# maxilevi/vits.cpp

Hardware: AMD Instinct MI355X
Metric: audio samples/sec end-to-end (ids -> fp32 PCM in HBM), vits-english architecture, batch=64 x 128 ids (higher is better)
Workload: dtype f32; 1 GPU; c3 b64x128 ref-mode f32 predicted-dur | vits-english = MMS-TTS arch, synthetic weights; batch_per_gpu=64, ids_per_utterance=128, parallelism=utterance-sharded x1

## Files before the change

### vits.cpp_amd/csrc/conv_mfma.hip

```cpp
#include <hip/hip_runtime.h>
#include <type_traits>

#include <algorithm>
#include <atomic>
#include <cmath>
#include <cstdint>
#include <cstdlib>
#include <cstring>

#include "kernels.h"

#ifndef VITS_CONV_PART
#define VITS_CONV_PART 0
#endif

namespace vits {

typedef float floatx16 __attribute__((ext_vector_type(16)));

constexpr int CK = 32;

struct ConvParams {
    const float* x;
    int64_t x_bs;
// ... 973 lines not shown
    const int t = t0 + col;
    if (EPI == EPI_STD) {
        float* yb = p.y + (int64_t)b * p.y_bs;
        float* y2b = p.y2 ? p.y2 + (int64_t)b * p.y_bs : nullptr;
        const float* rb = p.res ? p.res + (int64_t)b * p.r_bs : nullptr;
        const float* ab = p.acc ? p.acc + (int64_t)b * p.a_bs : nullptr;
#pragma unroll
        for (int r = 0; r < 4; ++r) {
            const int co = mtile * 32 + 16 * half + 4 * jg + r;
            if (co >= p.cout || t >= ncols) continue;
            float v = acc[r] + ep_bias[r];
            if (p.post_act == 1) v = v > 0.f ? v : 0.f;
            if (rb) v = ep_res[r] + v;
            if (ab) {
                v = ep_acc[r] + v;
                v = p.scale_div ? v / p.scale : v * p.scale;
            }
            if (p.post_act == 2) v = fmaxf(v, v * p.post_slope);
            yb[(int64_t)co * p.y_cs + t] = v;
            if (y2b) y2b[(int64_t)co * p.y_cs + t] = fmaxf(v, v * p.post_slope);
        }
    } else {
        float* ex = xs + (wm >> 1) * 256;
        __syncthreads();
        if (wm & 1) {
#pragma unroll
            for (int r = 0; r < 4; ++r) ex[r * 64 + lane] = acc[r];
        }
        __syncthreads();
        if (wm & 1) return;
        float* yb = p.y + (int64_t)b * p.y_bs;
        const int halfc = p.cout / 2;
#pragma unroll
        for (int r = 0; r < 4; ++r) {
            const int ch = (int)blockIdx.y * 32 + 16 * half + 4 * jg + r;
            if (ch >= halfc || t >= ncols) continue;
            yb[(int64_t)ch * p.y_cs + t] = wavenet_gate(acc[r] + ep_bias[r], ex[r * 64 + lane] + ep_b1[r]);
        }
    }
}

static int lat16_pitch(int span) { return span <= 4 ? 24 : span <= 20 ? 40 : span <= 52 ? 72 : 0; }
static hipError_t launch_lat16(const PackedConv& w, const ConvParams& p0, int ncols_max, int batch, hipStream_t s) {
    ConvParams p = p0;
    const int span = (w.kt - 1) * p.dil;
    const int pitch = lat16_pitch(span);
    if (!pitch || !w.wp_l16) return hipErrorInvalidValue;
    p.l16_fill4 = (reinterpret_cast<uintptr_t>(p.x) & 15) == 0 && (p.x_cs & 3) == 0 && (p.x_bs & 3) == 0;
    p.xw = pitch;
    p.kt_rt = w.kt;
    p.wl16 = w.wp_l16;
    size_t lds = ((size_t)w.nchunks + 1) * CK * pitch * sizeof(float);
    if (p.ln_gamma) lds += ((size_t)2 * 16 * 32 + 2 * (size_t)w.cin) * sizeof(float);
    dim3 grid((ncols_max + 15) / 16, (w.mtiles_used + 1) / 2, batch);
#define VITS_L16(E, PP)                                                                                                                          \
    do {                                                                                                                                         \
        static BigLdsOnce big;                                                                                                                   \
        if (lds > 64 * 1024 && big.needed()) {                                                                                                   \
            if (hipError_t e = hipFuncSetAttribute(reinterpret_cast<const void*>(&conv_lat16_kernel<E, PP>), hipFuncAttributeMaxDynamicSharedMemorySize, 160 * 1024)) \
                return e;                                                                                                                        \
            big.done();                                                                                                                          \
        }                                                                                                                                        \
        VITS_KLAUNCH((conv_lat16_kernel<E, PP>), grid, dim3(256), lds, s, p);                                                                    \
    } while (0)
    if (w.epi == EPI_GATE) {
        if (pitch != 24) return hipErrorInvalidValue;
        VITS_L16(EPI_GATE, 24);
    } else if (pitch == 24) {
        VITS_L16(EPI_STD, 24);
    } else if (pitch == 40) {
        VITS_L16(EPI_STD, 40);
    } else {
        VITS_L16(EPI_STD, 72);
    }
#undef VITS_L16
    return hipGetLastError();
}
#endif

struct ConvGroupParams {
    ConvParams m[3];
    int zend[3];
};
template <int DIL>
__global__ __launch_bounds__(320) VITS_WAVES_ATTR void conv_group_kernel(const ConvGroupParams g) {
    extern __shared__ __attribute__((aligned(16))) float xs_dyn[];
    const int z = blockIdx.z;
    if (z < g.zend[0]) conv_mfma_body<11, DIL, true, 2, 2, 2, 2, EPI_STD>(g.m[0], xs_dyn, blockIdx.x, blockIdx.y, z);
    else if (z < g.zend[1]) conv_mfma_body<7, DIL, true, 2, 2, 2, 2, EPI_STD>(g.m[1], xs_dyn, blockIdx.x, blockIdx.y, z - g.zend[0]);
    else conv_mfma_body<3, DIL, true, 2, 2, 2, 2, EPI_STD>(g.m[2], xs_dyn, blockIdx.x, blockIdx.y, z - g.zend[1]);
}

hipError_t make_conv_params(const PackedConv& w, const ConvCall& c, int tile, ConvParams& p);
struct TileShape {
    int wm, wn, mr, nr;
};
static TileShape tile_shape(int tile) {
    switch (tile) {
        case TILE_128x128: return {2, 2, 2, 2};
        case TILE_64x256: return {1, 4, 2, 2};
        case TILE_32x256: return {1, 4, 1, 2};
        case TILE_64x64: return {1, 4, 2, 1};
        case TILE_LAT16:
        case TILE_NARROW: return {4, 1, 1, 1};
        default: return {1, 4, 1, 1};
    }
}

#if VITS_CONV_PART == 0
int choose_conv_tile(int rows, int epi, int t_hint) {
    const int narrow = kernel_knobs().narrow_tiles;
    const bool small_t = t_hint <= 128 || (narrow && rows <= narrow);
    if (epi == EPI_GATE) return small_t ? TILE_64x64 : TILE_64x256;
    const int t128 = kernel_knobs().tile128;
    if (rows % 128 == 0 && t128) return TILE_128x128;
    if (rows % 64 == 0) return small_t ? TILE_64x64 : TILE_64x256;
    return small_t ? TILE_32x64 : TILE_32x256;
}

std::vector<float> pack_conv_weights(const float* w, int cout, int cin, int k, int epi, int ct_stride, int* rows_out, int* mtiles_used_out,
                                     int* mtiles_out, int* nchunks_out) {
    const int bm_tiles = 4;
    const int half = cout / 2;
    int rows, kt;
    if (epi == EPI_CONVT) {
        rows = cout * ct_stride;
        kt = k / ct_stride;
    } else {
        rows = cout;
        kt = k;
    }
    int mtiles = (rows + 31) / 32;
    if (epi == EPI_GATE) mtiles = 2 * ((half + 31) / 32);
    *mtiles_used_out = mtiles;
    mtiles = (mtiles + bm_tiles - 1) / bm_tiles * bm_tiles;
    const int nchunks = (cin + CK - 1) / CK;
    std::vector<float> out((size_t)mtiles * nchunks * kt * (CK / 2) * 64, 0.f);
    for (int mt = 0; mt < mtiles; ++mt)
        for (int c = 0; c < nchunks; ++c)
            for (int j = 0; j < kt; ++j)
                for (int pr = 0; pr < CK / 2; ++pr)
                    for (int l = 0; l < 64; ++l) {
                        const int ci = c * CK + 2 * pr + (l >> 5);
                        const int r = l & 31;
                        float v = 0.f;
                        if (ci < cin) {
                            if (epi == EPI_STD) {
                                const int co = mt * 32 + r;
                                if (co < cout) v = w[((size_t)co * cin + ci) * k + j];
                            } else if (epi == EPI_GATE) {
                                const int ch = (mt / 2) * 32 + r;
                                const int co = (mt & 1) ? half + ch : ch;
                                if (ch < half) v = w[((size_t)co * cin + ci) * k + j];
                            } else {
                                const int rho = mt * 32 + r;
                                const int co = rho / ct_stride, ph = rho % ct_stride;
                                if (co < cout) v = w[((size_t)ci * cout + co) * k + ph + ct_stride * j];
                            }
                        }
                        const size_t idx = (((((size_t)mt * nchunks + c) * kt + j) * (CK / 8) + pr / 4) * 64 + l) * 4 + (pr & 3);
                        out[idx] = v;
                    }
    *rows_out = rows;
    *mtiles_out = mtiles;
    *nchunks_out = nchunks;
    return out;
}

bool conv_lat16_candidate(int epi, int kt, int cin) {
    return (epi == EPI_STD || (epi == EPI_GATE && kt == 5)) && (int64_t)kt * cin >= 64;
}

std::vector<float> repack_conv_weights_l16(const std::vector<float>& packed, int mtiles, int nchunks, int kt) {
    std::vector<float> out(packed.size() + 32 * 256, 0.f);
    const size_t G = (size_t)nchunks * kt;
    for (int mt = 0; mt < mtiles; ++mt)
        for (int half = 0; half < 2; ++half)
            for (size_t g = 0; g < G; ++g)
                for (int hq = 0; hq < 2; ++hq)
                    for (int l = 0; l < 64; ++l)
                        for (int sc = 0; sc < 4; ++sc) {
                            const int ci = 16 * hq + 4 * sc + (l >> 4);
                            const int pr = ci >> 1, par = ci & 1;
                            const size_t src = (((((size_t)mt * G + g) * (CK / 8)) + pr / 4) * 64 + (16 * half + (l & 15) + 32 * par)) * 4 + (pr & 3);
                            const size_t dst = (((((size_t)mt * 2 + half) * (2 * G)) + 2 * g + hq) * 64 + l) * 4 + sc;
                            out[dst] = packed[src];
                        }
    return out;
}

#endif

template <int KT, int DIL, bool DB, int EPI>
static hipError_t launch_tile(const PackedConv& w, int tile, const ConvParams& p, int ncols_max, int batch, hipStream_t s) {
    const TileShape ts = tile_shape(tile);
    const int bn = ts.wn * ts.nr * 32;
    const int bm_tiles = ts.wm * ts.mr;
    dim3 grid((ncols_max + bn - 1) / bn, (w.mtiles_used + bm_tiles - 1) / bm_tiles, batch);
    const size_t lds = DB ? (size_t)p.nbuf * CK * ((p.xw + 3 + VITS_XWP_GRAN - 1) / VITS_XWP_GRAN * VITS_XWP_GRAN) * sizeof(float) : (size_t)CK * p.xw * sizeof(float);
#define VITS_LAUNCH(WM, WN, MR, NR)                                                                                                   \
    do {                                                                                                                              \
        static BigLdsOnce big_lds_set;          \
        if (lds > 64 * 1024 && big_lds_set.needed()) {                                                                                        \
            hipError_t ea = hipFuncSetAttribute(reinterpret_cast<const void*>(&conv_mfma_kernel<KT, DIL, DB, WM, WN, MR, NR, EPI>),       \
                                                hipFuncAttributeMaxDynamicSharedMemorySize, 160 * 1024);                             \
            if (ea != hipSuccess) return ea;                                                                                          \
            big_lds_set.done();                                                                                                 \
        }                                                                                                                             \
        VITS_KLAUNCH((conv_mfma_kernel<KT, DIL, DB, WM, WN, MR, NR, EPI>), grid, dim3(DB ? 320 : 256), lds, s, p);                             \
    } while (0)
    switch (tile) {
        case TILE_128x128:
            if (EPI == EPI_GATE) return hipErrorInvalidValue;
            VITS_LAUNCH(2, 2, 2, 2);
            break;
        case TILE_64x256: VITS_LAUNCH(1, 4, 2, 2); break;
        case TILE_64x64: VITS_LAUNCH(1, 4, 2, 1); break;
        case TILE_32x256:
            if (EPI == EPI_GATE) return hipErrorInvalidValue;
            VITS_LAUNCH(1, 4, 1, 2);
            break;
        case TILE_NARROW:
            if constexpr (DB && DIL == 1 && ((EPI == EPI_STD && KT <= 3) || (EPI == EPI_GATE && KT == 5))) {
                VITS_LAUNCH(4, 1, 1, 1);
                break;
            } else {
                return hipErrorInvalidValue;
            }
        default:
            if (EPI == EPI_GATE) return hipErrorInvalidValue;
            VITS_LAUNCH(1, 4, 1, 1);
            break;
    }
#undef VITS_LAUNCH
    return hipGetLastError();
}

#define VITS_GO(K, D, E)                                                                     \
    do {                                                                                     \
        if ((D) != 0 && db) return launch_tile<K, D, (D) != 0, E>(w, tile, p, ncols_max, batch, s); \
        return launch_tile<K, D, false, E>(w, tile, p, ncols_max, batch, s);                 \
    } while (0)
#define VITS_LAUNCHER(K) hipError_t launch_conv_k##K(const PackedConv& w, int tile, const ConvParams& p, int ncols_max, int batch, hipStream_t s, bool db)
VITS_LAUNCHER(3);
VITS_LAUNCHER(7);
VITS_LAUNCHER(11);
#if VITS_CONV_PART == 1
VITS_LAUNCHER(3) {
    if (p.dil == 1) VITS_GO(3, 1, EPI_STD);
    if (p.dil == 3) VITS_GO(3, 3, EPI_STD);
    if (p.dil == 5) VITS_GO(3, 5, EPI_STD);
    VITS_GO(3, 0, EPI_STD);
}
#endif
#if VITS_CONV_PART == 2
VITS_LAUNCHER(7) {
    if (p.dil == 1) VITS_GO(7, 1, EPI_STD);
    if (p.dil == 3) VITS_GO(7, 3, EPI_STD);
    if (p.dil == 5) VITS_GO(7, 5, EPI_STD);
    VITS_GO(7, 0, EPI_STD);
}
#endif
#if VITS_CONV_PART == 3
VITS_LAUNCHER(11) {
    if (p.dil == 1) VITS_GO(11, 1, EPI_STD);
    if (p.dil == 3) VITS_GO(11, 3, EPI_STD);
    if (p.dil == 5) VITS_GO(11, 5, EPI_STD);
    VITS_GO(11, 0, EPI_STD);
}
#endif

#if VITS_CONV_PART == 4
bool conv_group_supported(const PackedConv& w, int dil) {
    return w.epi == EPI_STD && (w.kt == 11 || w.kt == 7 || w.kt == 3) && (dil == 1 || dil == 3 || dil == 5) && w.rows % 128 == 0 && w.cin % CK == 0;
}
hipError_t launch_conv_group(const PackedConv* const* w, const ConvCall* c, int n, hipStream_t s) {
    if (n < 1 || n > 3) return hipErrorInvalidValue;
    ConvGroupParams g;
    std::memset(&g, 0, sizeof(g));
    const int slot_kt[3] = {11, 7, 3};
    int have[3] = {-1, -1, -1};
    for (int i = 0; i < n; ++i) {
        if (!conv_group_supported(*w[i], c[i].dil) || c[i].dil != c[0].dil || c[i].batch != c[0].batch || w[i]->rows != w[0]->rows || c[i].tile >= 0) return hipErrorInvalidValue;
        const int slot = w[i]->kt == 11 ? 0 : w[i]->kt == 7 ? 1 : 2;
        if (have[slot] >= 0) return hipErrorInvalidValue;
        have[slot] = i;
    }
    int z = 0, ncols_max = 0;
    size_t lds = 0;
    for (int slot = 0; slot < 3; ++slot) {
        if (have[slot] >= 0) {
            const int i = have[slot];
            if (hipError_t e = make_conv_params(*w[i], c[i], TILE_128x128, g.m[slot])) return e;
            if (g.m[slot].oneshot) return hipErrorInvalidValue;
            if (g.m[slot].bias_rows) return hipErrorInvalidValue;
            g.m[slot].nbuf = 2;
            z += c[i].batch;
            ncols_max = std::max(ncols_max, c[i].t_out);
            const int xwp = (g.m[slot].xw + 3 + VITS_XWP_GRAN - 1) / VITS_XWP_GRAN * VITS_XWP_GRAN;
            lds = std::max(lds, (size_t)2 * CK * xwp * sizeof(float));
        }
        g.zend[slot] = z;
        (void)slot_kt;
    }
    dim3 grid((ncols_max + 127) / 128, w[0]->mtiles_used / 4, z);
#define VITS_GROUP_LAUNCH(D)                                                                                                              \
    do {                                                                                                                                  \
        static BigLdsOnce big_lds_set;                                                                                      \
        if (lds > 64 * 1024 && big_lds_set.needed()) {                                                            \
            hipError_t ea = hipFuncSetAttribute(reinterpret_cast<const void*>(&conv_group_kernel<D>), hipFuncAttributeMaxDynamicSharedMemorySize, 160 * 1024); \
            if (ea != hipSuccess) return ea;                                                                                              \
            big_lds_set.done();                                                                           \
        }                                                                                                                                 \
        VITS_KLAUNCH((conv_group_kernel<D>), grid, dim3(320), lds, s, g);                                                           \
    } while (0)
    if (c[0].dil == 1) VITS_GROUP_LAUNCH(1);
    else if (c[0].dil == 3) VITS_GROUP_LAUNCH(3);
    else VITS_GROUP_LAUNCH(5);
#undef VITS_GROUP_LAUNCH
    return hipGetLastError();
}
#endif

#if VITS_CONV_PART == 0
int resolve_conv_tile(const PackedConv& w, const ConvCall& c) {
    const int ncols_max = w.epi == EPI_CONVT ? c.t_in + 1 : c.t_out;
    int tile = c.tile >= 0 ? c.tile : choose_conv_tile(w.rows, w.epi, ncols_max);
    if (c.tile < 0 && w.epi == EPI_GATE) {
        const TileShape t2 = tile_shape(tile);
        const int64_t nb = (ncols_max + t2.wn * t2.nr * 32 - 1) / (t2.wn * t2.nr * 32);
        if (nb * ((w.mtiles_used + 1) / 2) * c.batch < 512) tile = TILE_64x64;
    }
    if (c.tile < 0 && w.epi != EPI_GATE) {
        auto blocks = [&](int tl) {
            const TileShape t2 = tile_shape(tl);
            const int64_t nb = (ncols_max + t2.wn * t2.nr * 32 - 1) / (t2.wn * t2.nr * 32);
            const int64_t mb = (w.mtiles_used + t2.wm * t2.mr - 1) / (t2.wm * t2.mr);
            return nb * mb * c.batch;
        };
        const int64_t min_blocks_env = kernel_knobs().min_blocks;
        const int64_t min_blocks = min_blocks_env > 0 ? min_blocks_env : (w.kt <= 3 ? 1024 : 512);
        if (blocks(tile) < min_blocks && (tile == TILE_128x128 || tile == TILE_64x256)) tile = TILE_64x64;
        if (blocks(tile) < min_blocks && (tile == TILE_64x64 || tile == TILE_32x256)) tile = TILE_32x64;
    }
    if (c.tile < 0 && w.epi != EPI_CONVT) {
        const bool no_narrow = kernel_knobs().no_narrow;
        const int dil_eff = w.kt == 1 ? 1 : c.dil;
        const bool shape_ok = dil_eff == 1 && ((w.epi == EPI_STD && w.kt <= 3) || (w.epi == EPI_GATE && w.kt == 5));
        const TileShape t2 = tile_shape(tile);
        const int64_t nb = (int64_t)((ncols_max + t2.wn * t2.nr * 32 - 1) / (t2.wn * t2.nr * 32)) * ((w.mtiles_used + t2.wm * t2.mr - 1) / (t2.wm * t2.mr)) * c.batch;
        const int narrow_k1 = kernel_knobs().narrow_k1;
        const bool k1_short = narrow_k1 > 0 && w.epi == EPI_STD && w.kt == 1 && ncols_max <= narrow_k1;
        if (!no_narrow && shape_ok && (nb <= 128 || k1_short)) tile = TILE_NARROW;
        const int pitch16 = lat16_pitch((w.kt - 1) * dil_eff);
        const int64_t waves32 = (int64_t)((ncols_max + 31) / 32) * w.mtiles_used * c.batch;
        const bool tiny = tile == TILE_NARROW && nb <= 128;
        const bool unfilled = w.epi == EPI_STD && w.kt >= 3 && dil_eff >= 1 && waves32 <= kernel_knobs().lat16_max_waves;
        if ((tiny || unfilled) && !kernel_knobs().no_lat16 && w.wp_l16 && pitch16 && (w.epi == EPI_STD || pitch16 == 24) &&
            ((size_t)w.nchunks + 1) * CK * pitch16 * 4 <= 150 * 1024)
            tile = TILE_LAT16;
    }
    return tile;
}

hipError_t make_conv_params(const PackedConv& w, const ConvCall& c, int tile, ConvParams& p) {
    p.x = c.x.p;
    p.x_bs = c.x.bs;
    p.x_cs = c.x.cs;
    p.y = c.y.p;
    p.y_bs = c.y.bs;
    p.y_cs = c.y.cs;
    p.res = c.res.p;
    p.r_bs = c.res.bs;
    p.r_cs = c.res.cs;
    p.acc = c.acc.p;
    p.a_bs = c.acc.bs;
    p.a_cs = c.acc.cs;
    p.wp = w.wp;
    p.bias = w.bias;
    p.bias_rows = w.bias_rs ? c.spk : nullptr;
    p.bias_rs = w.bias_rs;
    p.len_in = c.len_in;
    p.len_out = c.len_out;
    p.t_in = c.t_in;
    p.t_out = c.t_out;
    p.cin = w.cin;
    p.cout = w.cout;
    p.rows = w.rows;
    p.nchunks = w.nchunks;
    p.mtiles = w.mtiles;
    p.pre_act = c.pre_act;
    p.slope = c.slope;
    p.post_act = c.post_act;
    p.post_slope = c.post_slope;
    p.y2 = c.y2;
    p.scale = c.scale;
    p.scale_div = c.scale_div;
    p.ct_stride = w.ct_stride;
    p.ct_crop = c.ct_crop;
    p.kt_rt = w.kt;
    p.wl16 = w.wp_l16;
    p.l16_fill4 = 0;
    p.ln_gamma = c.ln_gamma;
    p.ln_beta = c.ln_beta;
    p.ln_eps = c.ln_eps;
    p.ln_out = c.ln_out.p;
    p.lo_bs = c.ln_out.bs;
    p.lo_cs = c.ln_out.cs;
    const int ncols_max = w.epi == EPI_CONVT ? c.t_in + 1 : c.t_out;
    const TileShape ts = tile_shape(tile);
    const int bn = ts.wn * ts.nr * 32;
    if (w.epi == EPI_CONVT) {
        p.dil = -1;
        p.pad_l = 0;
    } else {
        p.dil = w.kt == 1 ? 1 : c.dil;
        p.pad_l = c.pad_l;
    }
    const int span = (w.kt - 1) * p.dil;
    p.lds_off = span < 0 ? -span : 0;
    p.xw = bn + (span < 0 ? -span : span);
    if ((size_t)2 * CK * p.xw * 4 > 160 * 1024) return hipErrorInvalidValue;
    {
        const int nbuf_env = kernel_knobs().nbuf;
// ... 71 lines not shown
```

### vits.cpp_amd/csrc/engine_vocoder.cpp

```cpp
#include "engine_internal.h"

namespace vits {

int Engine::run_vocoder_window16(Call& c, WinCtx& w) {
    std::string& err = c.err;
    const int B = c.B, n_up = c.n_up;
    const int F = hp.flow_size;
    const bool refmode = c.refmode;
    Call::S2& s2 = c.s2;
    const std::vector<int>& sts = c.sts;
    const int lws = c.lws;
    const int Lw = w.Lw;
    const int* const* d_len = w.d_len;
    const std::vector<int>& smax = w.smax;
    const std::vector<int64_t>& ssum = w.ssum;
    const TensorRef zwin = w.zwin, pre = w.pre, wv = w.wv;
    const int emit_lo = w.emit_lo;
    const int* emit_hi = w.emit_hi;
    const float final_slope = w.final_slope;
    auto TR = make_ref;
    auto R16 = [](float* base, int channels, int stride) {
        Ref16 r;
        r.p = reinterpret_cast<uint16_t*>(base);
        r.ts = stride;
// ... 430 lines not shown
        }
        bool splitrb[3] = {false, false, false};
        bool any_split = false;
        for (size_t j = 0; j < nk && j < 3 && split_on() && s2.sp_u; ++j) {
            const ResBlockW& R = U.rbs[j];
            bool f = !fusedrb[j] && C >= 128;
            for (size_t d = 0; d < R.dil.size() && f; ++d) f = conv_split_supported(R.c1[d], R.dil[d]) && conv_split_supported(R.c2[d], 1);
            splitrb[j] = f;
            any_split = any_split || f;
        }
        auto SR = [&](uint16_t* ptr) {
            Split3Ref r;
            r.p = ptr;
            r.ts = sts[st_out];
            r.ps = (int64_t)C * sts[st_out];
            r.bs = 3 * r.ps;
            return r;
        };
        if (any_split) {
            prof.begin("split_planes", 0, 10.0 * (double)C * (double)ssum[st_out], stream);
            HIP_OK(launch_split_planes(bu, C, d_len[st_out], B, smax[st_out], hp.lrelu, SR(s2.sp_u), stream));
            prof.end(stream);
        }
        bool sum3 = false;
        auto run_block = [&](size_t j, hipStream_t sj) -> int {
            const ResBlockW& R = U.rbs[j];
            const PackedConv* w1[3] = {&R.c1[0], &R.c1[1], &R.c1[2]};
            const PackedConv* w2[3] = {&R.c2[0], &R.c2[1], &R.c2[2]};
            RbBlock32Call f;
            f.x = bu;
            f.lens = d_len[st_out];
            f.batch = B;
            f.tmax = smax[st_out];
            f.slope = hp.lrelu;
            f.y = bsum;
            if (j > 0) f.acc = bsum;
            if (j + 1 == nk) {
                if (refmode) {
                    f.scale = (float)(1.0 / (double)nk);
                    f.scale_div = 0;
                } else {
                    f.scale = (float)nk;
                    f.scale_div = 1;
                }
                if (i + 1 < n_up) {
                    f.post_act = 2;
                    f.post_slope = hp.lrelu;
                }
            } else {
                f.scale = 1.f;
            }
            if (sum3) {
                f.y = TR(s2.by[j], C, sts[st_out]);
                f.acc = TensorRef();
                f.scale = 1.f;
                f.scale_div = 0;
                f.post_act = 0;
            }
            if (prof.on) {
                char full[160];
                std::snprintf(full, sizeof(full), "hifigan_resblock_block|k%d|d135|b%d|e0|c%dx%d", R.k, C, C, C);
                const double n_out = (double)C * (double)ssum[st_out];
                double bytes = 4.0 * n_out * (2 + (f.acc.p ? 1 : 0));
                for (size_t d = 0; d < R.dil.size(); ++d) bytes += (double)R.c1[d].bytes + (double)R.c2[d].bytes;
                prof.begin(full, 3.0 * 2.0 * 2.0 * (double)C * C * R.k * (double)ssum[st_out], bytes, sj, true);
            }
            HIP_OK(launch_rbblock32(w1, w2, f, sj));
            prof.end(sj);
            return 0;
        };
        bool grouped = exact32 && !any_split && !knobs.no_rb_group && nk >= 2 && nk <= 3 && knobs.rb_streams > 1 && (prof.on || knobs.rb_group_always);
        {
            int members = 0, seen = 0;
            for (size_t j = 0; j < nk && grouped; ++j) {
                const ResBlockW& R = U.rbs[j];
                if (R.dil != U.rbs[0].dil) grouped = false;
                if (fusedrb[j]) continue;
                const int bit = R.k == 11 ? 1 : R.k == 7 ? 2 : R.k == 3 ? 4 : 0;
                if (!bit || (seen & bit)) grouped = false;
                seen |= bit;
                ConvCall shape;
                shape.batch = B;
                shape.t_in = shape.t_out = smax[st_out];
                for (size_t d = 0; d < R.dil.size() && grouped; ++d)
                    grouped = conv_group_supported(R.c1[d], R.dil[d]) && conv_group_supported(R.c2[d], 1) && resolve_conv_tile(R.c1[d], shape) == TILE_128x128;
                ++members;
            }
            grouped = grouped && members >= 2;
        }
        const bool par = knobs.rb_streams > 1 && nk >= 2 && nk <= 3 && !prof.on;
        auto bufq = [&](size_t j) { return (par || grouped) ? (int)j : 0; };
        auto mk_c1 = [&](size_t j, size_t d) {
            const ResBlockW& R = U.rbs[j];
            const int q = bufq(j);
            TensorRef by = TR(s2.by[q], C, sts[st_out]), bt = TR(s2.bt[q], C, sts[st_out]), byl = TR(s2.byl[q], C, sts[st_out]);
            TensorRef resid = d == 0 ? bu : by;
            ConvCall c1;
            c1.x = lcopy ? (d > 0 ? byl : bul) : resid;
            c1.y = bt;
            c1.len_in = c1.len_out = d_len[st_out];
            c1.batch = B;
            c1.t_in = c1.t_out = smax[st_out];
            c1.sum_in = c1.sum_out = ssum[st_out];
            c1.dil = R.dil[d];
            c1.pad_l = (R.k * R.dil[d] - R.dil[d]) / 2;
            c1.pre_act = lcopy ? 0 : 1;
            c1.slope = hp.lrelu;
            c1.post_act = 2;
            c1.post_slope = hp.lrelu;
            if (j < 3 && splitrb[j]) {
                c1.x = TensorRef();
                c1.xs3 = d > 0 ? SR(s2.sp_y[q]) : SR(s2.sp_u);
                c1.y = TensorRef();
                c1.ys3 = SR(s2.sp_t[q]);
                c1.ys3_slope = hp.lrelu;
                c1.pre_act = 0;
                c1.post_act = 0;
            }
            return c1;
        };
        auto mk_c2 = [&](size_t j, size_t d) {
            const ResBlockW& R = U.rbs[j];
            const size_t nd = R.dil.size();
            const int q = bufq(j);
            TensorRef by = TR(s2.by[q], C, sts[st_out]), bt = TR(s2.bt[q], C, sts[st_out]), byl = TR(s2.byl[q], C, sts[st_out]);
            ConvCall c2 = mk_c1(j, d);
            c2.x = bt;
            c2.pre_act = 0;
            c2.post_act = 0;
            c2.y2 = (d + 1 < nd && lcopy) ? byl.p : nullptr;
            c2.dil = 1;
            c2.pad_l = (R.k - 1) / 2;
            c2.res = d == 0 ? bu : by;
            if (j < 3 && splitrb[j]) {
                c2.y = by;
                c2.xs3 = SR(s2.sp_t[q]);
                c2.y2 = nullptr;
                c2.ys3 = Split3Ref();
                if (d + 1 < nd) {
                    c2.ys3 = SR(s2.sp_y[q]);
                    c2.ys3_slope = hp.lrelu;
                }
            }
            if (d + 1 < nd) c2.y = by;
            else {
                c2.y = bsum;
                if (j > 0) c2.acc = bsum;
                if (j + 1 == nk) {
                    if (refmode) {
                        c2.scale = (float)(1.0 / (double)nk);
                        c2.scale_div = 0;
                    } else {
                        c2.scale = (float)nk;
                        c2.scale_div = 1;
                    }
                } else {
                    c2.scale = 1.f;
                }
                if (j + 1 == nk && i + 1 < n_up) {
                    c2.post_act = 2;
                    c2.post_slope = hp.lrelu;
                }
                if (sum3) {
                    c2.y = by;
                    c2.acc = TensorRef();
                    c2.scale = 1.f;
                    c2.scale_div = 0;
                    c2.post_act = 0;
// ... 3 lines not shown
        };
        auto run_fused = [&](size_t j, size_t d, hipStream_t sj) -> int {
            const ResBlockW& R = U.rbs[j];
            const size_t nd = R.dil.size();
            const int q = bufq(j);
            TensorRef by = TR(s2.by[q], C, sts[st_out]), bt = TR(s2.bt[q], C, sts[st_out]);
            const bool last = d + 1 == nd;
            RbPair32Call f;
            f.x = d == 0 ? bu : ((d & 1) ? by : bt);
            f.lens = d_len[st_out];
            f.batch = B;
            f.tmax = smax[st_out];
            f.dil = R.dil[d];
            f.slope = hp.lrelu;
            if (!last) {
                f.y = (d & 1) ? bt : by;
            } else {
                f.y = bsum;
                if (j > 0) f.acc = bsum;
                if (j + 1 == nk) {
                    if (refmode) {
                        f.scale = (float)(1.0 / (double)nk);
                        f.scale_div = 0;
                    } else {
                        f.scale = (float)nk;
                        f.scale_div = 1;
                    }
                    if (i + 1 < n_up) {
                        f.post_act = 2;
                        f.post_slope = hp.lrelu;
                    }
                } else {
                    f.scale = 1.f;
                }
                if (sum3) {
                    f.y = by;
                    f.acc = TensorRef();
                    f.scale = 1.f;
                    f.scale_div = 0;
                    f.post_act = 0;
                }
            }
            if (prof.on) {
                char full[160];
                std::snprintf(full, sizeof(full), "hifigan_resblock_pair|k%d|d%d|f%d|e0|c%dx%d", R.k, R.dil[d], C, C, C);
                const double n_out = (double)C * (double)ssum[st_out];
                prof.begin(full, 2.0 * 2.0 * (double)C * C * R.k * (double)ssum[st_out], 4.0 * n_out * (3 + (f.acc.p ? 1 : 0)) + (double)R.c1[d].bytes + (double)R.c2[d].bytes, sj, true);
            }
            HIP_OK(launch_rbpair32(R.c1[d], R.c2[d], f, sj));
            prof.end(sj);
            return 0;
        };
        if (grouped) {
            const size_t nd = U.rbs[0].dil.size();
            bool any_fused = false;
            for (size_t j = 0; j < nk; ++j) any_fused = any_fused || (fusedrb[j] && !blockrb[j]);
            hipStream_t sf = (any_fused && !prof.on) ? side_[0] : stream;
            if (sf != stream) {
                HIP_OK(hipEventRecord(ev_fork_, stream));
                HIP_OK(hipStreamWaitEvent(sf, ev_fork_, 0));
            }
            for (size_t j = 0; j < nk; ++j)
                if (fusedrb[j] && !blockrb[j])
                    for (size_t d = 0; d + 1 < nd; ++d)
                        if (run_fused(j, d, sf)) return -1;
            if (sf != stream) HIP_OK(hipEventRecord(ev_done_[0], sf));
            auto run_group = [&](size_t d, bool second) -> int {
                const PackedConv* gw[3];
                ConvCall gc[3];
                int n = 0;
                double flop = 0, bytes = 0;
                for (size_t j = 0; j < nk; ++j) {
                    if (fusedrb[j]) continue;
                    const ResBlockW& R = U.rbs[j];
                    gw[n] = second ? &R.c2[d] : &R.c1[d];
                    gc[n] = second ? mk_c2(j, d) : mk_c1(j, d);
                    const ConvCall& cc = gc[n];
                    flop += conv_flops(*gw[n], cc, ssum[st_out]);
                    bytes += 4.0 * ((double)C * ssum[st_out] * (2 + (cc.res.p ? 1 : 0) + (cc.acc.p ? 1 : 0) + (cc.y2 ? 1 : 0))) + (double)gw[n]->bytes;
                    ++n;
                }
                if (prof.on) {
                    char full[160];
                    std::snprintf(full, sizeof(full), "hifigan_resblock_group%d|kG|d%d|G0|e0|c%dx%d", n, second ? 1 : U.rbs[0].dil[d], C, C);
                    prof.begin(full, flop, bytes, stream, true);
                }
                HIP_OK(launch_conv_group(gw, gc, n, stream));
                prof.end(stream);
                return 0;
            };
            for (size_t d = 0; d < nd; ++d) {
                if (run_group(d, false)) return -1;
                if (d + 1 < nd && run_group(d, true)) return -1;
            }
            if (sf != stream) HIP_OK(hipStreamWaitEvent(stream, ev_done_[0], 0));
            for (size_t j = 0; j < nk; ++j) {
                if (blockrb[j]) {
                    if (run_block(j, stream)) return -1;
                } else if (fusedrb[j]) {
                    if (run_fused(j, nd - 1, stream)) return -1;
                } else {
                    HIP_OK(conv("hifigan_resblock_conv", U.rbs[j].c2[nd - 1], mk_c2(j, nd - 1), stream));
                }
            }
            cur = bsum;
            continue;
        }
        {
            bool odd = true;
            for (size_t j = 0; j < nk; ++j) odd = odd && (U.rbs[j].dil.size() & 1);
            sum3 = par && odd && !any_split && !knobs.kernel.no_rb_sum3 && !knobs.kernel.no_rb_sum3_f32 && w.ssum[0] < knobs.rb32_sum3_max_frames;
        }
        if (par) {
            HIP_OK(hipEventRecord(ev_fork_, stream));
            for (size_t j = 1; j < nk; ++j) HIP_OK(hipStreamWaitEvent(side_[j - 1], ev_fork_, 0));
        }
        for (size_t jj = 0; jj < nk; ++jj) {
            const size_t j = sum3 ? nk - 1 - jj : jj;
            const ResBlockW& R = U.rbs[j];
            const size_t nd = R.dil.size();
            hipStream_t sj = par && jj > 0 ? side_[jj - 1] : stream;
            const bool fuse_rb = j < 3 ? fusedrb[j] : false;
            if (j < 3 && blockrb[j]) {
                if (par && j > 0 && !sum3) HIP_OK(hipStreamWaitEvent(sj, ev_done_[j - 1], 0));
                if (run_block(j, sj)) return -1;
                if (par) HIP_OK(hipEventRecord(ev_done_[j], sj));
                continue;
            }
            for (size_t d = 0; d < nd; ++d) {
                const bool last = d + 1 == nd;
                if (!fuse_rb) HIP_OK(conv("hifigan_resblock_conv", R.c1[d], mk_c1(j, d), sj));
                if (par && last && j > 0 && !sum3) HIP_OK(hipStreamWaitEvent(sj, ev_done_[j - 1], 0));
                if (fuse_rb) {
                    if (run_fused(j, d, sj)) return -1;
                } else {
                    HIP_OK(conv("hifigan_resblock_conv", R.c2[d], mk_c2(j, d), sj));
                }
                if (par && last) HIP_OK(hipEventRecord(ev_done_[j], sj));
            }
        }
        if (par) HIP_OK(hipStreamWaitEvent(stream, ev_done_[nk - 1], 0));
        if (sum3) {
            for (size_t j = 0; j + 1 < nk; ++j) HIP_OK(hipStreamWaitEvent(stream, ev_done_[j], 0));
            const bool div = !refmode;
            const bool act = i + 1 < n_up;
            prof.begin("hifigan_resblock_sum", 0, 4.0 * (nk + 1) * (double)C * (double)ssum[st_out], stream);
            HIP_OK(launch_rb_sum3_std(TR(s2.by[0], C, sts[st_out]), TR(s2.by[1], C, sts[st_out]), nk > 2 ? TR(s2.by[2], C, sts[st_out]) : TensorRef(), bsum, C, d_len[st_out], B, smax[st_out],
                                      div ? (float)nk : (float)(1.0 / (double)nk), div ? 1 : 0, act ? 2 : 0, hp.lrelu, stream));
            prof.end(stream);
        }
        cur = bsum;
    }
    prof.begin("hifigan_conv_post_tanh", 2.0 * dec_post_cin_ * dec_post_k_ * (double)ssum[n_up], 4.0 * (dec_post_cin_ + 1) * (double)ssum[n_up], stream);
    HIP_OK(launch_conv_post(cur, dec_post_w_, dec_post_cin_, dec_post_k_, final_slope, pre, wv, d_len[n_up], B, smax[n_up], stream, emit_lo, emit_hi, arith_now_));
    prof.end(stream);
    (void)F;
    return 0;
}

}
```

### vits.cpp_amd/csrc/kernels.h

```cpp
#pragma once
#include <hip/hip_runtime.h>
#include <hip/hip_ext.h>

#include <atomic>
#include <cstdint>
#include <cstdlib>
#include <vector>

namespace vits {

struct KernelKnobs {
    int narrow_tiles = 64;
    int tile128 = 1;
    int min_blocks = 0;
    bool no_narrow = false;
    int narrow_k1 = 1 << 30;
    int nbuf = 0;
    bool no_oneshot = false;
    int db_min = 1;
    int t16_tile0 = 0;
    bool no_convt16s = false;
    bool convt16s_all = false;
    bool no_convt16l = false;
    bool no_att_lat = false;
    bool att_valu = false;
    int att_nw = 0;
    int att_short = 512;
    int ln_tw = 32;
    bool rbb_c128 = true;
    int rbb_c64k11 = -1;
    int rbb_stream_tiles = -1;
    int rbb_stream_min_blocks = 1536;
    int fuse16_maxc = 256;
    bool fuse32_c128 = true;
    int wn16_ncw = 1;
    int flow_ncw = 2;
    int convt16_r128 = 0;
    int convt16_split_max = 64;
    bool no_rbb_group3_c64 = false;
    bool no_rbb_group3 = false;
    bool no_rb_sum3_f32 = false;
    bool rb_sum3_in_order = false;
    bool rb_sum3_block_only = false;
    bool no_rb_sum3 = false;
    int rb16_narrow_max = 128;
    int flow_narrow_max = 96;
    bool no_ln_fuse = false;
    bool no_dds_lat = false;
    int dds_lat_max_blocks = 96;
    int lat16h_group_shape = 21;
    bool no_lat16h_group = false;
    bool no_lat16h_pre = false;
    bool no_lat16h = false;
    int lat16h_max_tiles = 2048;
    int lat16h_max_tiles_c128 = 0;
    int lat16h_shape = 21;
    bool no_lat16 = false;
    int lat16_max_waves = 768;
    static KernelKnobs from_env() {
        KernelKnobs k;
        auto num = [](const char* name, int& v) {
            if (const char* e = getenv(name)) v = atoi(e);
        };
        auto flag = [](const char* name, bool& v) { v = getenv(name) != nullptr; };
        num("VITS_NARROW_TILES", k.narrow_tiles);
        flag("VITS_NO_DDS_LAT", k.no_dds_lat);
        flag("VITS_NO_LN_FUSE", k.no_ln_fuse);
        flag("VITS_NO_RB_SUM3", k.no_rb_sum3);
        flag("VITS_RB_SUM3_BLOCK_ONLY", k.rb_sum3_block_only);
        flag("VITS_RB_SUM3_IN_ORDER", k.rb_sum3_in_order);
        flag("VITS_NO_RB_SUM3_F32", k.no_rb_sum3_f32);
        flag("VITS_NO_RBB_GROUP3", k.no_rbb_group3);
        flag("VITS_NO_RBB_GROUP3_C64", k.no_rbb_group3_c64);
        num("VITS_DDS_LAT_MAX_BLOCKS", k.dds_lat_max_blocks);
        num("VITS_TILE128", k.tile128);
        num("VITS_MIN_BLOCKS", k.min_blocks);
        flag("VITS_NO_NARROW", k.no_narrow);
        num("VITS_NARROW_K1", k.narrow_k1);
        num("VITS_NBUF", k.nbuf);
        flag("VITS_NO_ONESHOT", k.no_oneshot);
        num("VITS_DB_MIN", k.db_min);
        num("VITS_T16_TILE0", k.t16_tile0);
        flag("VITS_NO_CONVT16S", k.no_convt16s);
        flag("VITS_CONVT16S_ALL", k.convt16s_all);
        flag("VITS_NO_CONVT16L", k.no_convt16l);
        flag("VITS_ATT_VALU", k.att_valu);
        flag("VITS_NO_ATT_LAT", k.no_att_lat);
        num("VITS_ATT_NW", k.att_nw);
        num("VITS_ATT_SHORT", k.att_short);
        num("VITS_LN_TW", k.ln_tw);
        if (const char* e = getenv("VITS_RBB_C128")) k.rbb_c128 = atoi(e) != 0;
        num("VITS_RBB_C64K11", k.rbb_c64k11);
        num("VITS_RBB_STREAM_TILES", k.rbb_stream_tiles);
        num("VITS_RBB_STREAM_MIN_BLOCKS", k.rbb_stream_min_blocks);
        num("VITS_FUSE16_MAXC", k.fuse16_maxc);
        if (const char* e = getenv("VITS_FUSE32_C128")) k.fuse32_c128 = atoi(e) != 0;
        num("VITS_WN16_NCW", k.wn16_ncw);
        num("VITS_FLOW_NCW", k.flow_ncw);
        num("VITS_FLOW_NARROW_MAX", k.flow_narrow_max);
        num("VITS_RB16_NARROW_MAX", k.rb16_narrow_max);
        num("VITS_CONVT16_SPLIT_MAX", k.convt16_split_max);
        num("VITS_CONVT16_R128", k.convt16_r128);
        flag("VITS_NO_LAT16", k.no_lat16);
        flag("VITS_NO_LAT16H", k.no_lat16h);
        flag("VITS_NO_LAT16H_PRE", k.no_lat16h_pre);
        flag("VITS_NO_LAT16H_GROUP", k.no_lat16h_group);
        num("VITS_LAT16H_GROUP_SHAPE", k.lat16h_group_shape);
        num("VITS_LAT16H_MAX_TILES", k.lat16h_max_tiles);
        num("VITS_LAT16H_MAX_TILES_C128", k.lat16h_max_tiles_c128);
        num("VITS_LAT16H_SHAPE", k.lat16h_shape);
        num("VITS_LAT16_MAX_WAVES", k.lat16_max_waves);
        return k;
    }
};
namespace detail {
inline thread_local const KernelKnobs* tl_kernel_knobs = nullptr;
}
inline const KernelKnobs& kernel_knobs() {
    if (detail::tl_kernel_knobs) return *detail::tl_kernel_knobs;
    static const KernelKnobs process_default = KernelKnobs::from_env();
    return process_default;
}
struct KernelKnobsScope {
    const KernelKnobs* prev;
    explicit KernelKnobsScope(const KernelKnobs* k) : prev(detail::tl_kernel_knobs) { detail::tl_kernel_knobs = k; }
    ~KernelKnobsScope() { detail::tl_kernel_knobs = prev; }
    KernelKnobsScope(const KernelKnobsScope&) = delete;
    KernelKnobsScope& operator=(const KernelKnobsScope&) = delete;
};

struct BigLdsOnce {
    std::atomic<uint64_t> mask{0};
    static uint64_t bit() {
        int d = 0;
        (void)hipGetDevice(&d);
        return 1ull << (d & 63);
    }
    bool needed() const { return !(mask.load(std::memory_order_acquire) & bit()); }
    void done() { mask.fetch_or(bit(), std::memory_order_release); }
};

struct LaunchTimer {
    hipEvent_t start = nullptr, stop = nullptr;
    int launches = 0;
};
inline thread_local LaunchTimer vits_launch_timer;
#define VITS_KLAUNCH(kernel, grid, block, lds, stream, ...)                                                          \
    do {                                                                                                            \
        ::vits::LaunchTimer& lt_ = ::vits::vits_launch_timer;                                                       \
        if (lt_.start && lt_.launches++ == 0)                                                                       \
            hipExtLaunchKernelGGL(kernel, grid, block, lds, stream, lt_.start, lt_.stop, 0, __VA_ARGS__);           \
        else                                                                                                        \
            hipLaunchKernelGGL(kernel, grid, block, lds, stream, __VA_ARGS__);                                      \
    } while (0)

#ifdef __HIPCC__
__device__ __forceinline__ float wavenet_gate(float a, float s) { return tanhf(a) * (1.0f / (1.0f + expf(-s))); }
#endif

struct TensorRef {
    float* p = nullptr;
    int64_t bs = 0;
    int32_t cs = 0;
};

enum ConvEpilogue : int { EPI_STD = 0, EPI_GATE = 1, EPI_CONVT = 2 };
enum ConvTile : int {
    TILE_128x128 = 0,
    TILE_64x256 = 1,
    TILE_32x256 = 2,
    TILE_64x64 = 3,
    TILE_32x64 = 4,
    TILE_NARROW = 5,
    TILE_LAT16 = 6
};

struct PackedConv {
    float* wp = nullptr;
    float* bias = nullptr;
    int64_t bias_rs = 0;
    int cin = 0, cout = 0, kt = 0;
    int rows = 0;
    int mtiles = 0;
    int mtiles_used = 0;
    int nchunks = 0;
    int epi = EPI_STD;
    int ct_stride = 0;
    int64_t bytes = 0;
    uint16_t* wp16 = nullptr;
    float* wp_l16 = nullptr;
    int64_t bytes16 = 0;
    uint16_t* wps = nullptr;
    int64_t bytes_s = 0;
};

struct Ref16 {
    uint16_t* p = nullptr;
    int64_t bs = 0;
    int32_t ts = 0;
};

struct Split3Ref {
    uint16_t* p = nullptr;
    int64_t bs = 0;
    int64_t ps = 0;
    int32_t ts = 0;
};

struct ConvCall {
    TensorRef x, y, res, acc;
    const int* len_in = nullptr;
    const int* len_out = nullptr;
    const int* spk = nullptr;
    int batch = 1;
    int t_in = 0, t_out = 0;
    int64_t sum_in = -1, sum_out = -1;
    int dil = 1, pad_l = 0;
    int pre_act = 0;
    float slope = 0.f;
    int post_act = 0;
    float post_slope = 0.f;
    float* y2 = nullptr;
    float scale = 1.f;
    int scale_div = 0;
    int ct_crop = 0;
    int tile = -1;
    const float *ln_gamma = nullptr, *ln_beta = nullptr;
    float ln_eps = 0.f;
    TensorRef ln_out;
    Split3Ref xs3, ys3;
    float ys3_slope = 1.f;
};
bool conv_split_candidate(int epi, int kt, int cin, int cout);
bool pack_conv_weights_split(const float* w, int cout, int cin, int k, std::vector<uint16_t>& out);
bool conv_split_supported(const PackedConv& w, int dil);
hipError_t launch_conv_split(const PackedConv& w, const ConvCall& c, hipStream_t s);
hipError_t launch_split_planes(TensorRef x, int channels, const int* lens, int batch, int tmax, float slope, Split3Ref out, hipStream_t s);
bool conv_ln_on_load_ok(const PackedConv& w, const ConvCall& c);

std::vector<float> pack_conv_weights(const float* w, int cout, int cin, int k, int epi, int ct_stride, int* rows, int* mtiles_used, int* mtiles,
                                     int* nchunks);
bool conv_lat16_candidate(int epi, int kt, int cin);
std::vector<float> repack_conv_weights_l16(const std::vector<float>& packed, int mtiles, int nchunks, int kt);
int choose_conv_tile(int rows, int epi, int t_hint);
int resolve_conv_tile(const PackedConv& w, const ConvCall& c);
hipError_t launch_conv(const PackedConv& w, const ConvCall& c, hipStream_t s);
double conv_flops(const PackedConv& w, const ConvCall& c, int64_t total_cols);
bool conv_group_supported(const PackedConv& w, int dil);
hipError_t launch_conv_group(const PackedConv* const* w, const ConvCall* c, int n, hipStream_t s);

struct Conv16Call {
    Ref16 x;
    const int* len_in = nullptr;
    const int* len_out = nullptr;
    const int* spk = nullptr;
    int batch = 1, t_in = 0, t_out = 0, dil = 1, pad_l = 0;
    int post_act = 0;
    float post_slope = 0.f;
    float scale = 1.f;
    int scale_div = 0;
    int ct_crop = 0;
    int tile = -1;
    TensorRef y, res, acc;
    float* y2 = nullptr;
    float* yg = nullptr;
    const float* resg = nullptr;
    const float* accg = nullptr;
    int64_t g_bs = 0;
    int g_ts = 0;
    Ref16 y16;
    float y16_slope = 1.f;
    int64_t sum_in = -1, sum_out = -1;
};
struct RbPair16Call {
    Ref16 x;
    const int* lens = nullptr;
    int batch = 1, tmax = 0, dil = 1;
    float slope = 0.1f;
    float* yg = nullptr;
    const float* resg = nullptr;
    const float* accg = nullptr;
    int64_t g_bs = 0;
    int g_ts = 0;
    Ref16 y16;
    float y16_slope = 1.f;
    float scale = 1.f;
    int scale_div = 0;
};
bool rbpair16_supported(int channels, int kt, int dil);
struct RbBlock16Call {
    const float* y0 = nullptr;
    const int* lens = nullptr;
    int batch = 1, tmax = 0;
    float slope = 0.1f;
    float* yg = nullptr;
    const float* accg = nullptr;
    int64_t g_bs = 0;
    int g_ts = 0;
    Ref16 y16;
    float y16_slope = 1.f;
    float scale = 1.f;
    int scale_div = 0;
};
bool rbblock16_supported(int channels, int kt, const int* dils, int ndil, int batch, int tmax);
hipError_t launch_rbblock16(const PackedConv* const* c1, const PackedConv* const* c2, const RbBlock16Call& c, int arith, hipStream_t s);
bool rbblock16_group3_supported(int channels, const int* kts, int batch, int tmax);
hipError_t launch_rbblock16_group3(const PackedConv* const (*c1)[3], const PackedConv* const (*c2)[3], const RbBlock16Call* c, int arith, hipStream_t s);
hipError_t launch_rb_sum3(const float* y0, const float* y1, const float* y2, int channels, int64_t g_bs, int g_ts, const int* lens, int batch, int tmax, float scale, int scale_div,
                          float* yg, Ref16 y16, float y16_slope, int arith, hipStream_t s);
struct RbPair32Call {
    TensorRef x, y, acc;
    const int* lens = nullptr;
    int batch = 1, tmax = 0, dil = 1;
    float slope = 0.1f;
    float scale = 1.f;
    int scale_div = 0;
    int post_act = 0;
    float post_slope = 0.f;
};
bool rbpair32_supported(int channels, int kt, int dil);
struct RbBlock32Call {
    TensorRef x, y, acc;
    const int* lens = nullptr;
    int batch = 1, tmax = 0;
    float slope = 0.1f;
    float scale = 1.f;
    int scale_div = 0;
    int post_act = 0;
    float post_slope = 0.f;
};
bool rbblock32_supported(int channels, int kt, const int* dils, int ndil);
// ... 151 lines not shown
```

Baseline: 49.47 million samples/s.

## Add 128x256 and 256x128 MFMA conv tiles, including grouped resblock kernels

Adds two larger conv tile shapes (more MFMA fragments per wave) for the standard epilogue and kernel sizes 3/7/11, and lets the grouped HiFi-GAN resblock kernel use them when every member resolves to the same wide tile. The goal is more operand reuse per block and fewer LDS/global loads per FLOP on large-T vocoder convs. The default knob (-1) selects a rows-based policy that applies when enough blocks remain. The cost is higher register pressure, which may lower occupancy or cause spills. New compile parts 5 and 6 are also added for the grouped launchers.

```diff
diff --git a/vits.cpp_amd/csrc/conv_mfma.hip b/vits.cpp_amd/csrc/conv_mfma.hip
--- a/vits.cpp_amd/csrc/conv_mfma.hip
+++ b/vits.cpp_amd/csrc/conv_mfma.hip
@@ -1079,13 +1079,13 @@
     ConvParams m[3];
     int zend[3];
 };
-template <int DIL>
+template <int DIL, int MR, int NR>
 __global__ __launch_bounds__(320) VITS_WAVES_ATTR void conv_group_kernel(const ConvGroupParams g) {
     extern __shared__ __attribute__((aligned(16))) float xs_dyn[];
     const int z = blockIdx.z;
-    if (z < g.zend[0]) conv_mfma_body<11, DIL, true, 2, 2, 2, 2, EPI_STD>(g.m[0], xs_dyn, blockIdx.x, blockIdx.y, z);
-    else if (z < g.zend[1]) conv_mfma_body<7, DIL, true, 2, 2, 2, 2, EPI_STD>(g.m[1], xs_dyn, blockIdx.x, blockIdx.y, z - g.zend[0]);
-    else conv_mfma_body<3, DIL, true, 2, 2, 2, 2, EPI_STD>(g.m[2], xs_dyn, blockIdx.x, blockIdx.y, z - g.zend[1]);
+    if (z < g.zend[0]) conv_mfma_body<11, DIL, true, 2, 2, MR, NR, EPI_STD>(g.m[0], xs_dyn, blockIdx.x, blockIdx.y, z);
+    else if (z < g.zend[1]) conv_mfma_body<7, DIL, true, 2, 2, MR, NR, EPI_STD>(g.m[1], xs_dyn, blockIdx.x, blockIdx.y, z - g.zend[0]);
+    else conv_mfma_body<3, DIL, true, 2, 2, MR, NR, EPI_STD>(g.m[2], xs_dyn, blockIdx.x, blockIdx.y, z - g.zend[1]);
 }
 
 hipError_t make_conv_params(const PackedConv& w, const ConvCall& c, int tile, ConvParams& p);
@@ -1098,10 +1098,31 @@
         case TILE_64x256: return {1, 4, 2, 2};
         case TILE_32x256: return {1, 4, 1, 2};
         case TILE_64x64: return {1, 4, 2, 1};
+        case TILE_128x256: return {2, 2, 2, 4};
+        case TILE_256x128: return {2, 2, 4, 2};
         case TILE_LAT16:
         case TILE_NARROW: return {4, 1, 1, 1};
         default: return {1, 4, 1, 1};
     }
+}
+
+#ifdef VITS_MICRO_KT
+#define VITS_WIDE_TAPS_128x256(KT) true
+#define VITS_WIDE_TAPS_256x128(KT) true
+#else
+#define VITS_WIDE_TAPS_128x256(KT) ((KT) == 3 || (KT) == 7 || (KT) == 11)
+#define VITS_WIDE_TAPS_256x128(KT) ((KT) == 3 || (KT) == 7 || (KT) == 11)
+#endif
+#define VITS_WIDE_GROUP_128x256 (VITS_WIDE_TAPS_128x256(3) && VITS_WIDE_TAPS_128x256(7) && VITS_WIDE_TAPS_128x256(11))
+#define VITS_WIDE_GROUP_256x128 (VITS_WIDE_TAPS_256x128(3) && VITS_WIDE_TAPS_256x128(7) && VITS_WIDE_TAPS_256x128(11))
+#define VITS_WIDE_GROUP(tile) (((tile) == TILE_128x256 && VITS_WIDE_GROUP_128x256) || ((tile) == TILE_256x128 && VITS_WIDE_GROUP_256x128))
+static constexpr bool wide_tile_compiled(int tile, int kt, int dil) {
+    if (dil != 1 && dil != 3 && dil != 5) return false;
+    if (kt != 3 && kt != 7 && kt != 11) return false;
+    return tile == TILE_128x256 ? VITS_WIDE_TAPS_128x256(kt) : tile == TILE_256x128 ? VITS_WIDE_TAPS_256x128(kt) : false;
+}
+static bool wide_tile_supported(const PackedConv& w, int dil, int tile) {
+    return w.epi == EPI_STD && !w.bias_rs && wide_tile_compiled(tile, w.kt, dil) && w.cin % CK == 0 && w.rows % (tile == TILE_256x128 ? 256 : 128) == 0;
 }
 
 #if VITS_CONV_PART == 0
@@ -1211,6 +1232,20 @@
             if (EPI == EPI_GATE) return hipErrorInvalidValue;
             VITS_LAUNCH(2, 2, 2, 2);
             break;
+        case TILE_128x256:
+            if constexpr (DB && EPI == EPI_STD && wide_tile_compiled(TILE_128x256, KT, DIL)) {
+                VITS_LAUNCH(2, 2, 2, 4);
+                break;
+            } else {
+                return hipErrorInvalidValue;
+            }
+        case TILE_256x128:
+            if constexpr (DB && EPI == EPI_STD && wide_tile_compiled(TILE_256x128, KT, DIL)) {
+                VITS_LAUNCH(2, 2, 4, 2);
+                break;
+            } else {
+                return hipErrorInvalidValue;
+            }
         case TILE_64x256: VITS_LAUNCH(1, 4, 2, 2); break;
         case TILE_64x64: VITS_LAUNCH(1, 4, 2, 1); break;
         case TILE_32x256:
@@ -1267,12 +1302,52 @@
 }
 #endif
 
+#if VITS_CONV_PART >= 4
+template <int MR, int NR>
+static hipError_t launch_group_shape(int dil, dim3 grid, size_t lds, hipStream_t s, const ConvGroupParams& g) {
+#define VITS_GROUP_LAUNCH(D)                                                                                                              \
+    do {                                                                                                                                  \
+        static BigLdsOnce big_lds_set;                                                                                                    \
+        if (lds > 64 * 1024 && big_lds_set.needed()) {                                                                                    \
+            hipError_t ea = hipFuncSetAttribute(reinterpret_cast<const void*>(&conv_group_kernel<D, MR, NR>), hipFuncAttributeMaxDynamicSharedMemorySize, 160 * 1024); \
+            if (ea != hipSuccess) return ea;                                                                                              \
+            big_lds_set.done();                                                                                                           \
+        }                                                                                                                                 \
+        VITS_KLAUNCH((conv_group_kernel<D, MR, NR>), grid, dim3(320), lds, s, g);                                                         \
+    } while (0)
+    if (dil == 1) VITS_GROUP_LAUNCH(1);
+    else if (dil == 3) VITS_GROUP_LAUNCH(3);
+    else VITS_GROUP_LAUNCH(5);
+#undef VITS_GROUP_LAUNCH
+    return hipGetLastError();
+}
+hipError_t launch_group_128x256(int dil, dim3 grid, size_t lds, hipStream_t s, const ConvGroupParams& g);
+hipError_t launch_group_256x128(int dil, dim3 grid, size_t lds, hipStream_t s, const ConvGroupParams& g);
+#endif
 #if VITS_CONV_PART == 4
 bool conv_group_supported(const PackedConv& w, int dil) {
     return w.epi == EPI_STD && (w.kt == 11 || w.kt == 7 || w.kt == 3) && (dil == 1 || dil == 3 || dil == 5) && w.rows % 128 == 0 && w.cin % CK == 0;
 }
+int conv_group_tile(const PackedConv* const* w, const ConvCall* c, int n) {
+    int tile = -1;
+    bool same = true;
+    for (int i = 0; i < n; ++i) {
+        const int ti = resolve_conv_tile(*w[i], c[i]);
+        if (ti != TILE_128x128 && ti != TILE_128x256 && ti != TILE_256x128) return -1;
+        if (i > 0 && ti != tile) same = false;
+        tile = ti;
+    }
+    if (!same) return TILE_128x128;
+    for (int i = 0; i < n; ++i)
+        if (tile != TILE_128x128 && !(VITS_WIDE_GROUP(tile) && wide_tile_supported(*w[i], c[i].dil, tile))) return TILE_128x128;
+    return tile;
+}
 hipError_t launch_conv_group(const PackedConv* const* w, const ConvCall* c, int n, hipStream_t s) {
     if (n < 1 || n > 3) return hipErrorInvalidValue;
+    const int tile = conv_group_tile(w, c, n);
+    if (tile < 0) return hipErrorInvalidValue;
+    const TileShape tsh = tile_shape(tile);
+    const int bn = tsh.wn * tsh.nr * 32;
     ConvGroupParams g;
     std::memset(&g, 0, sizeof(g));
     const int slot_kt[3] = {11, 7, 3};
@@ -1288,7 +1363,7 @@
     for (int slot = 0; slot < 3; ++slot) {
         if (have[slot] >= 0) {
             const int i = have[slot];
-            if (hipError_t e = make_conv_params(*w[i], c[i], TILE_128x128, g.m[slot])) return e;
+            if (hipError_t e = make_conv_params(*w[i], c[i], tile, g.m[slot])) return e;
             if (g.m[slot].oneshot) return hipErrorInvalidValue;
             if (g.m[slot].bias_rows) return hipErrorInvalidValue;
             g.m[slot].nbuf = 2;
@@ -1300,26 +1375,36 @@
         g.zend[slot] = z;
         (void)slot_kt;
     }
-    dim3 grid((ncols_max + 127) / 128, w[0]->mtiles_used / 4, z);
-#define VITS_GROUP_LAUNCH(D)                                                                                                              \
-    do {                                                                                                                                  \
-        static BigLdsOnce big_lds_set;                                                                                      \
-        if (lds > 64 * 1024 && big_lds_set.needed()) {                                                            \
-            hipError_t ea = hipFuncSetAttribute(reinterpret_cast<const void*>(&conv_group_kernel<D>), hipFuncAttributeMaxDynamicSharedMemorySize, 160 * 1024); \
-            if (ea != hipSuccess) return ea;                                                                                              \
-            big_lds_set.done();                                                                           \
-        }                                                                                                                                 \
-        VITS_KLAUNCH((conv_group_kernel<D>), grid, dim3(320), lds, s, g);                                                           \
-    } while (0)
-    if (c[0].dil == 1) VITS_GROUP_LAUNCH(1);
-    else if (c[0].dil == 3) VITS_GROUP_LAUNCH(3);
-    else VITS_GROUP_LAUNCH(5);
-#undef VITS_GROUP_LAUNCH
-    return hipGetLastError();
+    dim3 grid((ncols_max + bn - 1) / bn, w[0]->mtiles_used / (tsh.wm * tsh.mr), z);
+    if (tile == TILE_128x256) return launch_group_128x256(c[0].dil, grid, lds, s, g);
+    if (tile == TILE_256x128) return launch_group_256x128(c[0].dil, grid, lds, s, g);
+    return launch_group_shape<2, 2>(c[0].dil, grid, lds, s, g);
+}
+#endif
+#if VITS_CONV_PART == 5
+hipError_t launch_group_128x256(int dil, dim3 grid, size_t lds, hipStream_t s, const ConvGroupParams& g) {
+#if VITS_WIDE_GROUP_128x256
+    return launch_group_shape<2, 4>(dil, grid, lds, s, g);
+#else
+    return hipErrorInvalidValue;
+#endif
+}
+#endif
+#if VITS_CONV_PART == 6
+hipError_t launch_group_256x128(int dil, dim3 grid, size_t lds, hipStream_t s, const ConvGroupParams& g) {
+#if VITS_WIDE_GROUP_256x128
+    return launch_group_shape<4, 2>(dil, grid, lds, s, g);
+#else
+    return hipErrorInvalidValue;
+#endif
 }
 #endif
 
 #if VITS_CONV_PART == 0
+static int wide_tile_policy(const PackedConv& w) {
+    if (w.rows % 256 == 0) return TILE_256x128;
+    return TILE_128x256;
+}
 int resolve_conv_tile(const PackedConv& w, const ConvCall& c) {
     const int ncols_max = w.epi == EPI_CONVT ? c.t_in + 1 : c.t_out;
     int tile = c.tile >= 0 ? c.tile : choose_conv_tile(w.rows, w.epi, ncols_max);
@@ -1337,6 +1422,15 @@
         };
         const int64_t min_blocks_env = kernel_knobs().min_blocks;
         const int64_t min_blocks = min_blocks_env > 0 ? min_blocks_env : (w.kt <= 3 ? 1024 : 512);
+        if (tile == TILE_128x128 && kernel_knobs().wide_tile != 0) {
+            const int knob = kernel_knobs().wide_tile;
+            const int64_t wide_min = min_blocks_env > 0 ? min_blocks_env : 512;
+            int want = -1;
+            if (knob == 1) want = TILE_128x256;
+            else if (knob == 2) want = TILE_256x128;
+            else want = wide_tile_policy(w);
+            if (want >= 0 && wide_tile_supported(w, c.dil, want) && blocks(want) >= wide_min) tile = want;
+        }
         if (blocks(tile) < min_blocks && (tile == TILE_128x128 || tile == TILE_64x256)) tile = TILE_64x64;
         if (blocks(tile) < min_blocks && (tile == TILE_64x64 || tile == TILE_32x256)) tile = TILE_32x64;
     }
diff --git a/vits.cpp_amd/csrc/engine_vocoder.cpp b/vits.cpp_amd/csrc/engine_vocoder.cpp
--- a/vits.cpp_amd/csrc/engine_vocoder.cpp
+++ b/vits.cpp_amd/csrc/engine_vocoder.cpp
@@ -536,8 +536,10 @@
                 ConvCall shape;
                 shape.batch = B;
                 shape.t_in = shape.t_out = smax[st_out];
-                for (size_t d = 0; d < R.dil.size() && grouped; ++d)
-                    grouped = conv_group_supported(R.c1[d], R.dil[d]) && conv_group_supported(R.c2[d], 1) && resolve_conv_tile(R.c1[d], shape) == TILE_128x128;
+                for (size_t d = 0; d < R.dil.size() && grouped; ++d) {
+                    const int t1 = resolve_conv_tile(R.c1[d], shape);
+                    grouped = conv_group_supported(R.c1[d], R.dil[d]) && conv_group_supported(R.c2[d], 1) && (t1 == TILE_128x128 || t1 == TILE_128x256 || t1 == TILE_256x128);
+                }
                 ++members;
             }
             grouped = grouped && members >= 2;
@@ -707,7 +709,7 @@
                 }
                 if (prof.on) {
                     char full[160];
-                    std::snprintf(full, sizeof(full), "hifigan_resblock_group%d|kG|d%d|G0|e0|c%dx%d", n, second ? 1 : U.rbs[0].dil[d], C, C);
+                    std::snprintf(full, sizeof(full), "hifigan_resblock_group%d|kG|d%d|G%d|e0|c%dx%d", n, second ? 1 : U.rbs[0].dil[d], std::max(0, conv_group_tile(gw, gc, n)), C, C);
                     prof.begin(full, flop, bytes, stream, true);
                 }
                 HIP_OK(launch_conv_group(gw, gc, n, stream));
diff --git a/vits.cpp_amd/csrc/kernels.h b/vits.cpp_amd/csrc/kernels.h
--- a/vits.cpp_amd/csrc/kernels.h
+++ b/vits.cpp_amd/csrc/kernels.h
@@ -12,6 +12,7 @@
 struct KernelKnobs {
     int narrow_tiles = 64;
     int tile128 = 1;
+    int wide_tile = -1;
     int min_blocks = 0;
     bool no_narrow = false;
     int narrow_k1 = 1 << 30;
@@ -74,6 +75,7 @@
         flag("VITS_NO_RBB_GROUP3_C64", k.no_rbb_group3_c64);
         num("VITS_DDS_LAT_MAX_BLOCKS", k.dds_lat_max_blocks);
         num("VITS_TILE128", k.tile128);
+        num("VITS_WIDE_TILE", k.wide_tile);
         num("VITS_MIN_BLOCKS", k.min_blocks);
         flag("VITS_NO_NARROW", k.no_narrow);
         num("VITS_NARROW_K1", k.narrow_k1);
@@ -172,7 +174,9 @@
     TILE_64x64 = 3,
     TILE_32x64 = 4,
     TILE_NARROW = 5,
-    TILE_LAT16 = 6
+    TILE_LAT16 = 6,
+    TILE_128x256 = 7,
+    TILE_256x128 = 8
 };
 
 struct PackedConv {
@@ -247,6 +251,7 @@
 hipError_t launch_conv(const PackedConv& w, const ConvCall& c, hipStream_t s);
 double conv_flops(const PackedConv& w, const ConvCall& c, int64_t total_cols);
 bool conv_group_supported(const PackedConv& w, int dil);
+int conv_group_tile(const PackedConv* const* w, const ConvCall* c, int n);
 hipError_t launch_conv_group(const PackedConv* const* w, const ConvCall* c, int n, hipStream_t s);
 
 struct Conv16Call {
```

New measurement: 47.83 million samples/s. -3.3%, worse.
